# mdnunez/bayesflow_nddms

Hardware: AMD Instinct MI355X
Metric: simulated DDM trials/sec at n_trials=300 dt=0.001 (basic_ddm_dc, max_steps=4000) (higher is better)
Workload: dtype f32

## Files before the change

### bayesflow_nddms_amd/build.py

```python
import hashlib
import os
import re
import shutil
import subprocess

_HERE = os.path.dirname(os.path.abspath(__file__))
SO_PATH = os.environ.get("NDDM_HIP_LIB") or os.path.join(_HERE, "libnddm_hip.so")
SOURCES = [os.path.join(_HERE, "csrc", "nddm_kernels.hip")]
HEADERS = [os.path.join(_HERE, "csrc", "nddm_rng.h"), os.path.join(_HERE, "csrc", "nddm_sim.h"), os.path.join(_HERE, "csrc", "nddm_queue.h"),
           os.path.join(_HERE, "csrc", "nddm_prepass.h"), os.path.join(_HERE, "csrc", "nddm_ratcliff.h"),
           os.path.join(_HERE, "csrc", "nddm_wiener.h"), os.path.join(_HERE, "csrc", "nddm_wiener_cdf.h"),
           os.path.join(_HERE, "csrc", "nddm_wiener_quantile.h"), os.path.join(_HERE, "csrc", "nddm_wiener_grad.h"),
           os.path.join(_HERE, "csrc", "nddm_wiener_survival_grad.h"),
           os.path.join(_HERE, "csrc", "nddm_wiener_marginal.h"), os.path.join(_HERE, "csrc", "nddm_wiener_marginal_grad.h"),
           os.path.join(_HERE, "csrc", "nddm_wiener_hmc.h"),
           os.path.join(_HERE, "csrc", "nddm_wiener_hmc_joint.h"),
           os.path.join(os.path.dirname(_HERE), "include", "nddm.h")]
HIPCC_FLAGS = ["-O3", "-ffp-contract=off", "--offload-arch=gfx950", "-fPIC", "-shared", "-std=c++17"]


def _hipcc():
    exe = shutil.which("hipcc") or "/opt/rocm/bin/hipcc"
    if not os.path.exists(exe):
        raise RuntimeError("hipcc not found: the HIP extension cannot be built")
    return exe


def source_hash():
    h = hashlib.sha256()
    for p in SOURCES + HEADERS:
        h.update(os.path.basename(p).encode() + b"\0")
        with open(p, "rb") as f:
            h.update(f.read())
        h.update(b"\0")
    h.update(" ".join(HIPCC_FLAGS).encode())
    return h.hexdigest()


def embedded_hash(path=None):
    path = path or SO_PATH
    try:
        with open(path, "rb") as f:
            m = re.search(rb"NDDM_SRC_HASH=([0-9a-f]{64})", f.read())
    except OSError:
        return None
    return m.group(1).decode() if m else None


def is_stale():
    if os.environ.get("NDDM_HIP_LIB"):
        return False
    if not os.path.exists(SO_PATH):
        return True
    return embedded_hash() != source_hash()


def hipcc_version():
    try:
        m = re.search(r"HIP version:\s*(\S+)", subprocess.run([_hipcc(), "--version"], capture_output=True, text=True, timeout=60).stdout)
        return m.group(1) if m else "unknown"
    except Exception:
        return "unknown"


def build_hip(force=False, verbose=False):
    if not force and not is_stale():
        return SO_PATH
    import fcntl
    with open(SO_PATH + ".lock", "w") as lock:
        fcntl.flock(lock, fcntl.LOCK_EX)
        if force or is_stale():
            tmp = f"{SO_PATH}.{os.getpid()}.tmp"
            cmd = [_hipcc()] + HIPCC_FLAGS + [f'-DNDDM_SOURCE_HASH="{source_hash()}"', f'-DNDDM_HIPCC_VERSION="{hipcc_version()}"', "-o", tmp] + SOURCES
            if verbose:
                print(" ".join(cmd))
            try:
                subprocess.check_call(cmd)
                os.replace(tmp, SO_PATH)
            finally:
                if os.path.exists(tmp):
                    os.remove(tmp)
    return SO_PATH


TRAIN_SO_PATH = os.path.join(_HERE, "libnddm_train.so")
TRAIN_SOURCES = [os.path.join(_HERE, "csrc", f) for f in ("train_kernels.hip", "train_sample.hip", "train_quantile.hip", "train_deepset.hip",
                                                          "train_update.hip", "train_importance.hip", "train_wquantile.hip", "train_psis.hip")]
TRAIN_HEADERS = [os.path.join(_HERE, "csrc", f) for f in ("train_flow.h", "train_quantile.h", "train_psis.h")]
TRAIN_SOURCE = TRAIN_SOURCES[0]


def train_source_hash():
    h = hashlib.sha256()
    for path in TRAIN_SOURCES + TRAIN_HEADERS:
        with open(path, "rb") as f:
            h.update(f.read())
    return h.hexdigest()


def train_is_stale():
    stamp = TRAIN_SO_PATH + ".srchash"
    try:
        with open(stamp) as f:
            return not os.path.exists(TRAIN_SO_PATH) or f.read().strip() != train_source_hash()
    except OSError:
        return True


def build_train(force=False, verbose=False):
    if not force and not train_is_stale():
        return TRAIN_SO_PATH
    import fcntl
    with open(TRAIN_SO_PATH + ".lock", "w") as lock:
        fcntl.flock(lock, fcntl.LOCK_EX)
        if force or train_is_stale():
            tmp = f"{TRAIN_SO_PATH}.{os.getpid()}.tmp"
            cmd = [_hipcc(), "-O3", "--offload-arch=gfx950", "-std=c++17", "-fPIC", "-shared", "-o", tmp] + TRAIN_SOURCES
            if verbose:
                print(" ".join(cmd))
            try:
                subprocess.check_call(cmd)
                os.replace(tmp, TRAIN_SO_PATH)
                with open(TRAIN_SO_PATH + ".srchash", "w") as f:
                    f.write(train_source_hash())
            finally:
                if os.path.exists(tmp):
                    os.remove(tmp)
    return TRAIN_SO_PATH


if __name__ == "__main__":
    print(build_hip(force=True, verbose=True))
    print(build_train(force=True, verbose=True))
```

### bayesflow_nddms_amd/csrc/nddm_sim.h

```cpp
#pragma once
#include <hip/hip_runtime.h>
#include <math.h>
#include <stdint.h>

#include "../../include/nddm.h"
#include "nddm_queue.h"
#include "nddm_rng.h"

namespace nddm {

constexpr int WAVE = 64;
constexpr int MAX_REJECT = 64;

typedef __attribute__((address_space(3))) uint16_t lds_u16;
typedef __attribute__((address_space(3))) uint32_t lds_u32;
typedef uint32_t u32v4 __attribute__((ext_vector_type(4)));
typedef uint32_t u32v2 __attribute__((ext_vector_type(2)));
typedef __attribute__((address_space(3))) u32v4 lds_u32v4;
typedef __attribute__((address_space(3))) u32v2 lds_u32v2;

template <int MODEL> struct ModelTraits;
template <> struct ModelTraits<NDDM_BASIC_DDM_DC>      { static constexpr int P = 5; static constexpr bool HAS_Z = false; static constexpr int TAU = 3; };
template <> struct ModelTraits<NDDM_SINGLE_TRIAL>      { static constexpr int P = 8; static constexpr bool HAS_Z = true;  static constexpr int TAU = 3; };
template <> struct ModelTraits<NDDM_SINGLE_TRIAL_ALT>  { static constexpr int P = 8; static constexpr bool HAS_Z = true;  static constexpr int TAU = 3; };
template <> struct ModelTraits<NDDM_ALPHA_NOT_SCALED>  { static constexpr int P = 6; static constexpr bool HAS_Z = false; static constexpr int TAU = 3; };
template <> struct ModelTraits<NDDM_EXPLICIT_BOUNDARY> { static constexpr int P = 4; static constexpr bool HAS_Z = true;  static constexpr int TAU = 2; };

struct SimArgs {
    const float *params;
    const float *bounds;
    float *out_trials;
    float *out_summary;
    float *out_ext;
    uint16_t *out_codes;
    long long B;
    int n_trials;
    int n_total;
    int tiles_per_set;
    unsigned long long *partials;
    const uint32_t *recs;
    int max_k;
    float dt;
    float sqrt_dt;
    float tscale;
    uint32_t k0, k1;
    int sets_per_chunk;
    int n_chunks;
    unsigned int *chunk_counter;
    int ring;
    int open_ahead;
    float ext_sigma;
    int ext_mode;
    unsigned long long *dbg;
    int dbg_waves, dbg_chunks;
    int res16;
    int refill_thresh;
    uint32_t ring_magic;
    int back_from;
    double dt64, sqrt_dt64;
};

typedef const __attribute__((address_space(4))) SimArgs *ArgsPtr;
__device__ __forceinline__ ArgsPtr fresh_args(ArgsPtr p)
{
    asm volatile("" : "+s"(p));
    return p;
}

template <bool FAST>
struct AuxStream {
    uint32_t trial, set_lo, c3, blk, kbase;
    u32x4 x;
    __device__ __forceinline__ AuxStream(uint32_t kbase_, uint32_t set_lo_, uint32_t set_hi28, uint32_t trial_)
        : trial(trial_), set_lo(set_lo_), c3(set_hi28 | 0x10000000u), blk(0xffffffffu), kbase(kbase_) {}
    __device__ __forceinline__ void block(uint32_t b)
    {
        if (b != blk) { x = philox4x32_10_lds(set_lo, trial, c3, b, kbase); blk = b; }
    }
    __device__ __forceinline__ void first_pair(float &z0, float &z1)
    {
        block(0u);
        float r, cs, sn;
        polar_pair<FAST>(x.x, x.y, r, cs, sn);
        r *= noise_unit<FAST>(1.0f);
        z0 = r * cs; z1 = r * sn;
    }
    __device__ __forceinline__ float normal(uint32_t a)
    {
        block(a >> 2);
        const bool second = (a & 2u) != 0u;
        float r, cs, sn;
        polar_pair<FAST>(second ? x.z : x.x, second ? x.w : x.y, r, cs, sn);
        r *= noise_unit<FAST>(1.0f);
        return r * ((a & 1u) ? sn : cs);
    }
};

__device__ __forceinline__ unsigned long long wave_sum(unsigned long long v)
{
#pragma unroll
    for (int off = 32; off > 0; off >>= 1) v += __shfl_xor(v, off, WAVE);
    return v;
}
__device__ __forceinline__ int wave_sum(int v)
{
#pragma unroll
    for (int off = 32; off > 0; off >>= 1) v += __shfl_xor(v, off, WAVE);
    return v;
}

__device__ __forceinline__ int fresh_lane(int lane)
{
    asm volatile("" : "+v"(lane));
    return lane;
}

__device__ __forceinline__ uint32_t lane_rank(unsigned long long mask)
{
    return __builtin_amdgcn_mbcnt_hi((uint32_t)(mask >> 32), __builtin_amdgcn_mbcnt_lo((uint32_t)mask, 0u));
}

__device__ __forceinline__ void finalize_summary(float *o, int n_up, int n_lo, int n_miss, unsigned long long sk,
                                                 unsigned long long sk2, unsigned long long sk_up,
                                                 unsigned long long sk2_up, long long sz, long long szz, int n_total,
                                                 float tscale, float tau)
{
    const double dtd = (double)tscale, taud = (double)tau;
    const double n_resp = (double)(n_up + n_lo);
    o[0] = (float)n_up; o[1] = (float)n_lo; o[2] = (float)n_miss;
    if (n_resp > 0) {
        const double mk = (double)sk / n_resp;
        const double vk = (double)sk2 / n_resp - mk * mk;
        o[3] = (float)(taud + dtd * mk);
        o[4] = (float)(dtd * dtd * vk);
    } else { o[3] = __builtin_nanf(""); o[4] = __builtin_nanf(""); }
    if (n_up > 0) {
        const double nu = (double)n_up;
        const double mk = (double)sk_up / nu;
        const double vk = (double)sk2_up / nu - mk * mk;
        o[5] = (float)(taud + dtd * mk);
        o[6] = (float)(dtd * dtd * vk);
    } else { o[5] = __builtin_nanf(""); o[6] = __builtin_nanf(""); }
    const double Nd = (double)n_total;
    const double mz = ((double)sz / 4294967296.0) / Nd;
    const double vz = ((double)szz / 16777216.0) / Nd - mz * mz;
    o[7] = (float)mz;
    o[8] = (float)(vz < 0 ? 0 : vz);
    o[9] = (float)(((double)n_up + 0.5 * (double)n_miss) / Nd);
}

enum { REC = 12, R_A = 0, R_B = 4, R_SET = 8, R_TAU = 9, R_GLO = 10, R_GHI = 11 };

__device__ __forceinline__ void make_record(int model, bool fast, bool f64, const float *row, float dt, float sqrt_dt, int set,
                                            unsigned long long gset, uint32_t *r)
{
    float drift = 0.0f, a = 0.0f, beta = 0.0f, sig_c = 1.0f, tau;
    float b0 = 0.0f, b1 = 0.0f, b2 = 0.0f;
    switch (model) {
    case NDDM_BASIC_DDM_DC: drift = row[0]; a = row[1]; beta = row[2]; tau = row[3]; sig_c = row[4]; break;
    case NDDM_SINGLE_TRIAL: drift = row[0]; beta = row[2]; tau = row[3]; sig_c = row[5]; b0 = row[6]; b1 = row[7]; b2 = row[2]; break;
    case NDDM_SINGLE_TRIAL_ALT: tau = row[3]; b0 = row[5]; b1 = row[6]; b2 = row[7]; break;
    case NDDM_ALPHA_NOT_SCALED: a = row[1]; beta = row[2]; tau = row[3]; sig_c = row[5]; b0 = row[4]; break;
    default: drift = row[0]; beta = row[1]; tau = row[2]; sig_c = row[3]; break;
    }
    const float unit = sqrt_dt * sig_c;
    const float inv_s = 1.0f / (fast ? noise_unit<true>(unit) : noise_unit<false>(unit));
    const float hv = 0.5f * a;
    float a0 = (drift * dt) * inv_s, a1 = inv_s, a2 = hv * inv_s, a3 = (a * beta - hv) * inv_s;
    if (model == NDDM_SINGLE_TRIAL) { a2 = row[4]; a3 = row[1]; }
    else if (model == NDDM_SINGLE_TRIAL_ALT) { a0 = row[0]; a1 = row[1]; a2 = row[2]; a3 = row[4]; }
    else if (model == NDDM_ALPHA_NOT_SCALED) { a0 = row[0]; }
    else if (model == NDDM_EXPLICIT_BOUNDARY) { a2 = beta; a3 = 0.0f; }
    if (f64) {
        a0 = drift; a1 = sig_c;
        if (model == NDDM_BASIC_DDM_DC) { a2 = a; a3 = beta; }
    }
    r[0] = __float_as_uint(a0); r[1] = __float_as_uint(a1); r[2] = __float_as_uint(a2); r[3] = __float_as_uint(a3);
    r[4] = __float_as_uint(b0); r[5] = __float_as_uint(b1); r[6] = __float_as_uint(b2); r[7] = 0u;
    r[8] = (uint32_t)set; r[9] = __float_as_uint(tau);
    r[R_GLO] = (uint32_t)gset; r[R_GHI] = (uint32_t)(gset >> 32) & 0x0fffffffu;
}

enum { D_A = 0, D_B = 4,
       D_SIC = 8, D_TAU = 9, D_TBASE = 10, D_VSET = 11,
       D_CA = 12, D_CB = 13, D_HP1K = 14, D_X1 = 15,
       D_C3 = 16, D_SETLO = 17,
       D_ZSUM = 20,
       D_SPARE = 20 };
constexpr int DV = 24;
static_assert(D_SIC == R_SET && D_TAU == R_TAU, "the LDS record starts with the loaded record");
constexpr int LDS_HEADER_DWORDS = 32;
__host__ __device__ constexpr bool model_has_latent(int model)
{
    return model == NDDM_SINGLE_TRIAL || model == NDDM_SINGLE_TRIAL_ALT || model == NDDM_ALPHA_NOT_SCALED;
}
constexpr int LATENT_FIFO = 128;
__host__ __device__ constexpr int lds_header_bytes(int model)
{
    return LDS_HEADER_DWORDS * 4 + (model_has_latent(model) ? LATENT_FIFO * 4 : 0);
}
__host__ __device__ constexpr int slot_stride_bytes(int tile_trials, int bytes_per_result)
{
    return DV * 4 + ((tile_trials * bytes_per_result + 15) & ~15);
}

template <int MODEL, bool FAST>
__device__ __forceinline__ void trial_latent(const u32v4 dA, const u32v4 dB, uint32_t set_lo, uint32_t c3, uint32_t trial,
                                             uint32_t kbase, float &latent, float &z)
{
    static_assert(MODEL == NDDM_SINGLE_TRIAL || MODEL == NDDM_SINGLE_TRIAL_ALT, "models with a per-trial latent");
    const float sd = MODEL == NDDM_SINGLE_TRIAL ? __uint_as_float(dA.z) : __uint_as_float(dA.w);
    const float mean = MODEL == NDDM_SINGLE_TRIAL ? __uint_as_float(dA.w) : __uint_as_float(dB.x);
    const float sigma1 = MODEL == NDDM_SINGLE_TRIAL ? __uint_as_float(dB.x) : __uint_as_float(dB.y);
    const float gamma = MODEL == NDDM_SINGLE_TRIAL ? __uint_as_float(dB.y) : __uint_as_float(dB.z);
    AuxStream<FAST> aux(kbase, set_lo, c3, trial);
    float z0, z1;
    aux.first_pair(z0, z1);
    float v = __builtin_fmaf(sd, z1, mean);
    for (uint32_t ai = 2; !(v > 0.0f) && ai <= MAX_REJECT; ++ai) v = __builtin_fmaf(sd, aux.normal(ai), mean);
    if (!(v > 0.0f)) v = fabsf(v);
    latent = v;
    z = __builtin_fmaf(sigma1, z0, gamma * v);
}

template <bool FAST>
__device__ __forceinline__ float latent_normal_f64(const u32v4 dA, uint32_t set_lo, uint32_t c3, uint32_t trial, uint32_t kbase)
{
    const double sd = (double)__uint_as_float(dA.z), mean = (double)__uint_as_float(dA.w);
    AuxStream<FAST> aux(kbase, set_lo, c3, trial);
    float z0, z;
    aux.first_pair(z0, z);
    double v = mean + sd * (double)z;
    for (uint32_t ai = 2; !(v > 0.0) && ai <= MAX_REJECT; ++ai) { z = aux.normal(ai); v = mean + sd * (double)z; }
    return z;
}

__device__ __forceinline__ void z_fixed_point(float z, long long &fz, long long &fzz)
{
    z = fminf(fmaxf(z, -262144.0f), 262144.0f);
    const uint32_t b = __float_as_uint(z);
    const uint32_t e = (b >> 23) & 0xffu;
    const uint32_t m = (b & 0x007fffffu) | 0x00800000u;
    const uint32_t s1 = 147u - e, s2 = 291u - 2u * e;
    const unsigned long long mag = ((unsigned long long)m << 29) >> (s1 < 63u ? s1 : 63u);
    fz = (b >> 31) ? -(long long)mag : (long long)mag;
    fzz = (long long)((((unsigned long long)m * m) << 15) >> (s2 < 63u ? s2 : 63u));
}

template <int CTRL, int ROW_MASK>
__device__ __forceinline__ uint32_t dpp_add(uint32_t v)
{
    return v + (uint32_t)__builtin_amdgcn_update_dpp(0, (int)v, CTRL, ROW_MASK, 0xf, false);
}
__device__ __forceinline__ uint32_t wave_sum_dpp(uint32_t v)
{
    v = dpp_add<0x111, 0xf>(v);
    v = dpp_add<0x112, 0xf>(v);
    v = dpp_add<0x114, 0xf>(v);
    v = dpp_add<0x118, 0xf>(v);
    v = dpp_add<0x142, 0xa>(v);
    v = dpp_add<0x143, 0xc>(v);
    return v;
}

__host__ __device__ constexpr int partial_words(bool has_zsum) { return has_zsum ? 7 : 5; }

template <int MODEL, bool FAST, bool SMALL, bool CODES>
__device__ __forceinline__ void flush_set(ArgsPtr Ap, int lane, long long vset, uint32_t *d, const void *res, uint32_t kbase)
{
    using T = ModelTraits<MODEL>;
    constexpr bool ZSUM = MODEL == NDDM_SINGLE_TRIAL || MODEL == NDDM_SINGLE_TRIAL_ALT;
    const float tau = __uint_as_float(d[D_TAU]);
    [[maybe_unused]] u32v4 dA = {0u, 0u, 0u, 0u}, dB = {0u, 0u, 0u, 0u};
    [[maybe_unused]] uint32_t set_lo = 0u, c3 = 0u;
    [[maybe_unused]] long long acc_z = 0, acc_zz = 0;
    if constexpr (ZSUM) {
        dA = *reinterpret_cast<const u32v4 *>(d + D_A); dB = *reinterpret_cast<const u32v4 *>(d + D_B);
        c3 = d[D_C3]; set_lo = d[D_SETLO];
    }
    const int N = Ap->n_trials;
    const int TPS = Ap->tiles_per_set;
    const long long set_in_call = TPS == 1 ? vset : vset / TPS;
    const int t0 = TPS == 1 ? 0 : (int)(vset - set_in_call * TPS) * N;
    const int n_here = (Ap->n_total - t0) < N ? (Ap->n_total - t0) : N;
    uint32_t cnt2 = 0, sk32 = 0, sk2_32 = 0, sk_up32 = 0, sk2_up32 = 0;
    int n_up = 0, n_lo = 0, n_miss = 0;
    unsigned long long sk = 0, sk2 = 0, sk_up = 0, sk2_up = 0;
    float2 *out = Ap->out_trials ? reinterpret_cast<float2 *>(Ap->out_trials) + set_in_call * Ap->n_total + t0 : nullptr;
    static_assert(!CODES || (SMALL && (MODEL == NDDM_BASIC_DDM_DC || MODEL == NDDM_ALPHA_NOT_SCALED)), "wire-format kernels");
    constexpr bool HAS_CODES = CODES;
    [[maybe_unused]] uint16_t *codes = nullptr;
    if constexpr (HAS_CODES) { if (Ap->out_codes) codes = Ap->out_codes + set_in_call * Ap->n_total + t0; }
    for (uint32_t j = (uint32_t)lane; j < (uint32_t)n_here; j += WAVE) {
        uint32_t k, code;
        if (SMALL || Ap->res16) {
            const uint32_t v = static_cast<const uint16_t *>(res)[j];
            k = v & 0x3fffu; code = v >> 14;
            if constexpr (HAS_CODES) { if (codes) codes[j] = (uint16_t)v; }
        } else {
            const uint32_t v = static_cast<const uint32_t *>(res)[j];
            k = v & 0x3fffffffu; code = v >> 30;
        }
        const float ch = code == 1u ? 1.0f : (code == 2u ? -1.0f : 0.0f);
        const float rt = __builtin_fmaf((float)k, Ap->tscale, tau);
        float2 o;
        if constexpr (MODEL == NDDM_BASIC_DDM_DC) { o.x = rt; o.y = ch; }
        else if constexpr (MODEL == NDDM_ALPHA_NOT_SCALED) { o.x = ch * rt; o.y = 0.5f * (ch + 1.0f); }
        else {
            o.x = ch * rt;
            if constexpr (ZSUM) {
                float latent;
                trial_latent<MODEL, FAST>(dA, dB, set_lo, c3, (uint32_t)(t0 + j), kbase, latent, o.y);
                if (Ap->out_summary) { long long fz, fzz; z_fixed_point(o.y, fz, fzz); acc_z += fz; acc_zz += fzz; }
            } else {
                o.y = out ? Ap->bounds[set_in_call * Ap->n_total + t0 + j] : 0.0f;
            }
        }
        if constexpr (MODEL == NDDM_EXPLICIT_BOUNDARY) { if (code == 3u) o.x = __builtin_nanf(""); }
        if (out) out[j] = o;
        if (Ap->out_summary) {
            if constexpr (SMALL) {
                const uint32_t up01 = __builtin_amdgcn_ubfe(0x2u, code, 1u), resp01 = __builtin_amdgcn_ubfe(0x6u, code, 1u);
                const uint32_t kr = __umul24(k, resp01), ku = __umul24(k, up01);
                cnt2 += up01 | (resp01 << 10);
                sk32 += kr; sk_up32 += ku;
                sk2_32 = __umul24(kr, k) + sk2_32; sk2_up32 = __umul24(ku, k) + sk2_up32;
            } else {
                const unsigned long long kk = (unsigned long long)k * k;
                if (code == 1u) { n_up++; sk += k; sk2 += kk; sk_up += k; sk2_up += kk; }
                else if (code == 2u) { n_lo++; sk += k; sk2 += kk; }
                else n_miss++;
            }
        }
    }
    if (Ap->out_summary) {
        unsigned long long *q = reinterpret_cast<unsigned long long *>(Ap->partials) + vset * partial_words(ZSUM);
        [[maybe_unused]] unsigned long long *zsum = reinterpret_cast<unsigned long long *>(d + D_ZSUM);
        if constexpr (ZSUM) {
            atomicAdd(zsum, (unsigned long long)acc_z);
            atomicAdd(zsum + 1, (unsigned long long)acc_zz);
        }
        if constexpr (SMALL) {
            cnt2 = wave_sum_dpp(cnt2);
            sk32 = wave_sum_dpp(sk32); sk_up32 = wave_sum_dpp(sk_up32);
            const uint32_t a_hi = wave_sum_dpp(sk2_32 >> 16), a_lo = wave_sum_dpp(sk2_32 & 0xffffu);
            const uint32_t u_hi = wave_sum_dpp(sk2_up32 >> 16), u_lo = wave_sum_dpp(sk2_up32 & 0xffffu);
            if (fresh_lane(lane) == WAVE - 1) {
                const uint32_t n_up = cnt2 & 1023u, n_resp = cnt2 >> 10;
                q[0] = (unsigned long long)n_up | ((unsigned long long)(n_resp - n_up) << 21) |
                       ((unsigned long long)((uint32_t)n_here - n_resp) << 42);
                q[1] = sk32; q[2] = ((unsigned long long)a_hi << 16) + a_lo;
                q[3] = sk_up32; q[4] = ((unsigned long long)u_hi << 16) + u_lo;
                if constexpr (ZSUM) { q[5] = zsum[0]; q[6] = zsum[1]; }
            }
        } else {
            n_up = wave_sum(n_up); n_lo = wave_sum(n_lo); n_miss = wave_sum(n_miss);
            sk = wave_sum(sk); sk2 = wave_sum(sk2); sk_up = wave_sum(sk_up); sk2_up = wave_sum(sk2_up);
            if (fresh_lane(lane) == 0) {
                q[0] = (unsigned long long)n_up | ((unsigned long long)n_lo << 21) | ((unsigned long long)n_miss << 42);
                q[1] = sk; q[2] = sk2; q[3] = sk_up; q[4] = sk2_up;
                if constexpr (ZSUM) { q[5] = zsum[0]; q[6] = zsum[1]; }
            }
        }
    }
    if constexpr (MODEL == NDDM_ALPHA_NOT_SCALED) {
        if (Ap->out_ext && fresh_lane(lane) == 0 && t0 == 0) {
            AuxStream<FAST> aux(kbase, d[D_SETLO], d[D_C3], 0xffffffffu);
            const float loc = (Ap->ext_mode == 0) ? Ap->params[set_in_call * T::P + 1] : 1.0f;
            Ap->out_ext[set_in_call] = __builtin_fmaf(Ap->ext_sigma, aux.normal(0), loc);
        }
    }
}

__device__ __forceinline__ int ring_slot(int t, int ring, uint32_t magic)
{
    const uint32_t q = (uint32_t)(((unsigned long long)(uint32_t)t * magic) >> 32);
    int r = t - (int)(q * (uint32_t)ring);
    return r >= ring ? r - ring : r;
}

__device__ __forceinline__ bool in_range(float w, float h)
{
    return __builtin_fabsf(w) < h;
}


template <int MODEL, bool FAST, bool CAP4, bool BRIDGE, bool SMALL, bool PACKED, bool VKEYS, bool CODES = false, bool F64 = false>
__global__ __launch_bounds__(WAVE) void sim_kernel(const SimArgs A)
{
    static_assert(!F64 || ((MODEL == NDDM_BASIC_DDM_DC || MODEL == NDDM_SINGLE_TRIAL) && !BRIDGE && !PACKED && !VKEYS && !CODES),
                  "NDDM_STATE_F64 kernels");
    using T = ModelTraits<MODEL>;
    constexpr int P = T::P;
    extern __shared__ uint32_t lds_raw[];

    const ArgsPtr Ak = (ArgsPtr)__builtin_amdgcn_kernarg_segment_ptr();
    const int lane = threadIdx.x;
    const int N = A.n_trials;

    if (lane < 10) { lds_raw[2 * lane] = A.k0 + (uint32_t)lane * 0x9E3779B9u; lds_raw[2 * lane + 1] = A.k1 + (uint32_t)lane * 0xBB67AE85u; }
    if (lane == 0) { lds_raw[28] = A.k0 + 2u * PHILOX_W0; lds_raw[29] = A.k1 + 2u * PHILOX_W1; lds_raw[30] = A.k0 + 3u * PHILOX_W0; }
    uint32_t kbase;
    {
        const uint32_t off = (uint32_t)(size_t)lds_raw;
        asm volatile("v_mov_b32 %0, %1" : "=v"(kbase) : "s"(off));
    }
    const int rshift = SMALL ? 1 : (BRIDGE ? 2 : (A.res16 ? 1 : 2));
    constexpr bool LATENT = model_has_latent(MODEL);
    const int stride = DV * 4 + (((N << rshift) + 15) & ~15);
    char *const slots = reinterpret_cast<char *>(lds_raw) + lds_header_bytes(MODEL);
    auto slot_rec = [&](int slot) { return reinterpret_cast<uint32_t *>(slots + slot * stride); };
    auto pack_slots = [&](int t) {
        const ArgsPtr R = fresh_args(Ak);
        const int s0 = ring_slot(t, R->ring, R->ring_magic);
        const int o0 = s0 * stride, o01 = (s0 + 1 == R->ring ? 0 : s0 + 1) * stride - o0;
        return (o0 & 0xffff) | (o01 << 16);
    };
    constexpr uint32_t SLOTS_OFF = lds_header_bytes(MODEL);
    constexpr uint32_t FIFO_OFF = LDS_HEADER_DWORDS * 4;
    [[maybe_unused]] int fifo_pos = 0, fifo_avail = 0;

    float w = 0.0f, h = 0.0f, mu_dt = 0.0f;
    [[maybe_unused]] double xe = 0.0, ab = 0.0, cdt = 0.0, sdc = 0.0;
    int k = 0;
    [[maybe_unused]] float ta = 0.0f, tb = 0.0f;
    [[maybe_unused]] uint32_t jraw = 0;
    uint32_t res_addr = 0;
    [[maybe_unused]] int tile = 0;
    bool invalid = false;
    unsigned long long has_m = 0ull, act_m = 0ull;
    constexpr int MAX_BLOCKS = 16;
    [[maybe_unused]] int cap_k = -1;
    PathCtr pc = {0u, 0u, 0u, 0u, 0u};
    [[maybe_unused]] PathKeys pkeys;
    if constexpr (VKEYS) pkeys.init(A.k0, A.k1);

    int tile_open = 0;
    int flushed = 0;
    int next_tile = 0, next_trial = 0;
    int to_retire = N;
    int chunk_set = 0, chunk_left = 0;
    int slot_pack = pack_slots(0);
    int dirty = 1;
    unsigned long long dbg_cnt = 0;
    unsigned long long *dbg_stamp = reinterpret_cast<unsigned long long *>(lds_raw + 20);
    if (lane == 0) {
        dbg_stamp[3] = 0;
        lds_raw[31] = blockIdx.x;
        if (Ak->dbg) { dbg_stamp[0] = __builtin_amdgcn_s_memtime(); dbg_stamp[1] = __builtin_amdgcn_s_memrealtime(); }
    }

    uint32_t pre = 0u;

    auto open_tiles = [&]() {
        const ArgsPtr R = fresh_args(Ak);
        while (tile_open < flushed + R->ring && tile_open <= next_tile + R->open_ahead) {
            const bool have_pre = chunk_left > 0;
            if (chunk_left <= 0) {
                if (chunk_left < 0) break;
                const bool from_back = __builtin_amdgcn_readfirstlane((int)lds_raw[31]) >= R->back_from;
                unsigned long long old = 0ull;
                if (fresh_lane(lane) == 0)
                    old = atomicAdd(reinterpret_cast<unsigned long long *>(R->chunk_counter), from_back ? QUEUE_BACK : QUEUE_FRONT);
                old = ((unsigned long long)(uint32_t)__builtin_amdgcn_readfirstlane((int)(old >> 32)) << 32) |
                      (uint32_t)__builtin_amdgcn_readfirstlane((int)(uint32_t)old);
                const long long pulled = queue_pull(old, R->n_chunks, from_back);
                const unsigned int c = (unsigned int)pulled;
                if (pulled < 0) {
                    chunk_left = -1;
                    if (fresh_lane(lane) == 0 && R->dbg) dbg_stamp[3] = __builtin_amdgcn_s_memrealtime();
                    break;
                }
                if (fresh_lane(lane) == 0 && R->dbg && c < (unsigned int)R->dbg_chunks)
                    R->dbg[8ll * R->dbg_waves + c] = __builtin_amdgcn_s_memrealtime();
                chunk_set = (int)c * R->sets_per_chunk;
                const long long left = R->B - (long long)chunk_set;
                chunk_left = (int)(left < R->sets_per_chunk ? left : R->sets_per_chunk);
            }
            const int slot = ring_slot(tile_open, R->ring, R->ring_magic);
            const int TPS = R->tiles_per_set;
            const int prow = TPS == 1 ? chunk_set : chunk_set / TPS;
            const int qt = chunk_set - prow * TPS;
            uint32_t rec = pre;
            if (!have_pre) rec = fresh_lane(lane) < REC ? R->recs[(long long)prow * REC + lane] : 0u;
            if (chunk_left > 1) {
                const int nrow = TPS == 1 ? chunk_set + 1 : (chunk_set + 1) / TPS;
                if (nrow != prow) pre = fresh_lane(lane) < REC ? R->recs[(long long)nrow * REC + lane] : 0u;
                else pre = rec;
            }
            const int sic = __builtin_amdgcn_readlane((int)rec, R_SET);
            const int vset = sic * TPS + qt;
            uint32_t *d = slot_rec(slot);
            if (lane < REC) d[lane] = rec;
            const uint32_t s_lo = (uint32_t)__builtin_amdgcn_readlane((int)rec, R_GLO);
            const uint32_t s_hi = (uint32_t)__builtin_amdgcn_readlane((int)rec, R_GHI);
            if (lane == 0) {
                d[D_VSET] = (uint32_t)vset;
                if constexpr (MODEL == NDDM_SINGLE_TRIAL || MODEL == NDDM_SINGLE_TRIAL_ALT) { d[D_ZSUM] = 0u; d[D_ZSUM + 1] = 0u; d[D_ZSUM + 2] = 0u; d[D_ZSUM + 3] = 0u; }
                PathSet ps;
                ps.init(s_lo, s_hi, R->k0, R->k1);
                d[D_CA] = ps.cA; d[D_CB] = ps.cB; d[D_HP1K] = ps.hP1k; d[D_X1] = ps.X1;
                d[D_SETLO] = s_lo;
                d[D_C3] = s_hi;
                d[D_TBASE] = (uint32_t)(qt * N);
            }
            chunk_set++; chunk_left--; tile_open++;
        }
    };

    while (true) {
        const unsigned long long fin_mask0 = has_m & ~act_m;
        if (__builtin_amdgcn_inverse_ballot_w64(fin_mask0)) {
            uint32_t code = invalid ? 3u : (w >= h ? 1u : (w <= -h ? 2u : 0u));
            if constexpr (F64) code = xe >= ab ? 1u : (xe <= 0.0 ? 2u : 0u);
            uint32_t tfix = (uint32_t)k;
            if constexpr (BRIDGE) {
                const bool started = fmaxf(ta, tb) > 0.0f;
                const bool stepped = started && k < A.max_k;
                code = (stepped || !started) ? (w >= 0.0f ? 1u : 2u) : 0u;
                const uint32_t jit = (k & 1) ? ((jraw >> 16) & 0xffu) : (jraw & 0xffu);
                tfix = (((uint32_t)k + (stepped ? 1u : 0u)) << 8) - (stepped ? jit : 0u);
            }
            if (SMALL || rshift == 1) *reinterpret_cast<lds_u16 *>(res_addr + (SLOTS_OFF + DV * 4)) = (uint16_t)(tfix | (code << 14));
            else *reinterpret_cast<lds_u32 *>(res_addr + (SLOTS_OFF + DV * 4)) = tfix | (code << 30);
        }
        has_m &= ~fin_mask0;
        to_retire -= (int)__popcll(fin_mask0);
        if (to_retire <= 0) {
            __syncthreads();
            while (flushed < tile_open) {
                if (next_tile <= flushed) break;
                const int fslot = ring_slot(flushed, fresh_args(Ak)->ring, fresh_args(Ak)->ring_magic);
                if constexpr (SMALL) {
                    const uint32_t fsb = (uint32_t)(fslot * stride) + kbase;
                    if (__builtin_amdgcn_ballot_w64(res_addr - fsb < (uint32_t)stride) & has_m) break;
                } else {
                    if (__builtin_amdgcn_ballot_w64(tile == flushed) & has_m) break;
                }
                uint32_t *const d = slot_rec(fslot);
                const int set_in_call = __builtin_amdgcn_readfirstlane((int)d[D_VSET]);
                flush_set<MODEL, FAST, SMALL, CODES>(fresh_args(Ak), lane, (long long)set_in_call, d, d + DV, kbase);
                flushed++;
                to_retire += N;
                dirty = 1;
            }
            __syncthreads();
        }
        if (dirty) {
            dirty = 0;
            if (tile_open <= next_tile + fresh_args(Ak)->open_ahead && tile_open < flushed + fresh_args(Ak)->ring && chunk_left >= 0) {
                open_tiles();
                __syncthreads();
            }
            if (flushed == tile_open && chunk_left < 0) break;
        }
        {
            const unsigned long long want_mask = ~has_m;
            int tr = next_trial + (int)lane_rank(want_mask);
            int tl = next_tile;
            while (tr >= N) { tr -= N; tl++; }
            const unsigned long long ok_mask = want_mask & __builtin_amdgcn_ballot_w64(tl < tile_open);
            const int off0 = slot_pack & 0xffff, off01 = slot_pack >> 16;
            const int tile0 = next_tile;
            if constexpr (LATENT) {
                const int n_ok = (int)__popcll(ok_mask);
                if (n_ok > fifo_avail) {
                    int btr = next_trial + fifo_avail + lane, btl = next_tile;
                    while (btr >= N) { btr -= N; btl++; }
                    const unsigned long long bmask = __builtin_amdgcn_ballot_w64(btl < tile_open);
                    if (__builtin_amdgcn_inverse_ballot_w64(bmask)) {
                        const uint32_t bsb = (uint32_t)(__mul24(btl - tile0, off01) + off0) + kbase;
                        const lds_u32v4 *const bq = reinterpret_cast<const lds_u32v4 *>(bsb + SLOTS_OFF);
                        const u32v4 dA = bq[D_A / 4];
                        [[maybe_unused]] const u32v4 dB = bq[D_B / 4];
                        const u32v4 dS = bq[D_SIC / 4];
                        const u32v2 sw = *reinterpret_cast<const lds_u32v2 *>(bsb + SLOTS_OFF + D_C3 * 4);
                        const uint32_t btrial = (uint32_t)btr + dS.z;
                        float v;
                        if constexpr (MODEL == NDDM_ALPHA_NOT_SCALED) {
                            AuxStream<FAST> aux(kbase, sw.y, sw.x, btrial);
                            v = (__builtin_fmaf(__uint_as_float(dB.x), aux.normal(0), __uint_as_float(dA.x)) * fresh_args(Ak)->dt) * __uint_as_float(dA.y);
                        } else if constexpr (F64) {
                            v = latent_normal_f64<FAST>(dA, sw.y, sw.x, btrial, kbase);
                        } else {
                            float z_unused;
                            trial_latent<MODEL, FAST>(dA, dB, sw.y, sw.x, btrial, kbase, v, z_unused);
                        }
                        *reinterpret_cast<__attribute__((address_space(3))) float *>(
                            kbase + FIFO_OFF + (((uint32_t)(fifo_pos + fifo_avail + lane) & (LATENT_FIFO - 1)) << 2)) = v;
                    }
                    fifo_avail += (int)__popcll(bmask);
                }
            }
            next_trial += (int)__popcll(ok_mask);
            if (next_trial >= N) {
                const int ring_bytes = fresh_args(Ak)->ring * stride;
                int o0 = slot_pack & 0xffff, o01 = slot_pack >> 16;
                while (next_trial >= N) {
                    next_trial -= N; next_tile++;
                    o0 += o01;
                    o01 = o0 + stride == ring_bytes ? -o0 : stride;
                }
                slot_pack = (o0 & 0xffff) | (o01 << 16);
                dirty = 1;
            }
            has_m |= ok_mask;
            if (__builtin_amdgcn_inverse_ballot_w64(ok_mask)) {
#ifdef NDDM_EXTRA_REFILL_VALU
                { uint32_t dummy = (uint32_t)lane;
#pragma unroll
                  for (int e = 0; e < NDDM_EXTRA_REFILL_VALU; ++e) asm volatile("v_xor_b32 %0, 0x55, %0" : "+v"(dummy)); }
#endif
                const ArgsPtr H = fresh_args(Ak);
                if constexpr (!SMALL) tile = tl;
                const uint32_t sb = (uint32_t)(__mul24(tl - tile0, off01) + off0) + kbase;
                res_addr = sb + ((uint32_t)tr << rshift);
                const lds_u32v4 *const rq = reinterpret_cast<const lds_u32v4 *>(sb + SLOTS_OFF);
                const lds_u32 *const rw = reinterpret_cast<const lds_u32 *>(sb + SLOTS_OFF);
                const u32v4 d0 = rq[D_A / 4];
                const u32v4 d1 = rq[D_CA / 4];
                const u32v4 d2 = rq[D_SIC / 4];
                const float a0 = __uint_as_float(d0.x), a1 = __uint_as_float(d0.y), a2 = __uint_as_float(d0.z),
                            a3 = __uint_as_float(d0.w);
                const uint32_t trial = (uint32_t)tr + d2.z;
                [[maybe_unused]] float latent = 0.0f;
                if constexpr (LATENT)
                    latent = *reinterpret_cast<const __attribute__((address_space(3))) float *>(
                        kbase + FIFO_OFF + (((uint32_t)fifo_pos + lane_rank(want_mask)) & (LATENT_FIFO - 1)) * 4u);
                invalid = false;
                if constexpr (F64) {
                    double beta64;
                    if constexpr (MODEL == NDDM_BASIC_DDM_DC) { ab = (double)a2; beta64 = (double)a3; }
                    else {
                        ab = (double)a3 + (double)a2 * (double)latent;
                        if (!(ab > 0.0)) ab = __builtin_fabs(ab);
                        beta64 = (double)__uint_as_float(rw[D_B + 2]);
                    }
                    xe = ab * beta64;
                    cdt = (double)a0 * H->dt64;
                    sdc = H->sqrt_dt64 * (double)a1;
                    if constexpr (FAST) sdc *= 1.1774100225154747;
                } else if constexpr (MODEL == NDDM_BASIC_DDM_DC) {
                    mu_dt = a0; h = a2; w = a3;
                } else if constexpr (MODEL == NDDM_SINGLE_TRIAL) {
                    const float a = latent;
                    const float hv = 0.5f * a;
                    mu_dt = a0;
                    h = hv * a1;
                    w = (a * __uint_as_float(rw[D_B + 2]) - hv) * a1;
                } else if constexpr (MODEL == NDDM_SINGLE_TRIAL_ALT) {
                    const float sig_c = latent;
                    const float inv_t = 1.0f / noise_unit<FAST>(H->sqrt_dt * sig_c);
                    const float hv = 0.5f * a1;
                    mu_dt = (a0 * H->dt) * inv_t;
                    h = hv * inv_t;
                    w = (a1 * a2 - hv) * inv_t;
                } else if constexpr (MODEL == NDDM_ALPHA_NOT_SCALED) {
                    mu_dt = latent;
                    h = a2; w = a3;
                } else if constexpr (MODEL == NDDM_EXPLICIT_BOUNDARY) {
                    const float a = trial < (uint32_t)H->n_total ? H->bounds[(long long)d2.x * H->n_total + trial] : 1.0f;
                    invalid = !(a >= 0.0f);
                    const float hv = 0.5f * a;
                    mu_dt = a0;
                    h = invalid ? 0.0f : hv * a1;
                    w = (a * a2 - hv) * a1;
                }
                const uint4 kq = *reinterpret_cast<const uint4 *>(lds_raw + 28);
                pc.init(d1.x, d1.y, d1.z, d1.w, trial, kq.x, kq.y, kq.z);
                k = 0;
                if constexpr (BRIDGE) { ta = h - __builtin_fabsf(w); tb = ta; jraw = 0u; }
            }
            if constexpr (LATENT) { const int n_ok = (int)__popcll(ok_mask); fifo_pos += n_ok; fifo_avail -= n_ok; }
            if constexpr (BRIDGE) act_m = __builtin_amdgcn_ballot_w64(ta > 0.0f) & __builtin_amdgcn_ballot_w64(k < A.max_k) & has_m;
            else if constexpr (F64) act_m = __builtin_amdgcn_ballot_w64(xe > 0.0) & __builtin_amdgcn_ballot_w64(xe < ab) & __builtin_amdgcn_ballot_w64(k < A.max_k) & has_m;
            else if constexpr (CAP4 && !PACKED) {
                const int max_k = fresh_args(Ak)->max_k;
                act_m = max_k > 0 ? __builtin_amdgcn_ballot_w64(in_range(w, h)) & has_m : 0ull;
                const int near_from = A.refill_thresh < WAVE ? max_k - 4 * MAX_BLOCKS : (int)0x80000000;
                cap_k = (__builtin_amdgcn_ballot_w64(k >= near_from) & has_m) ? max_k : -1;
            }
            else act_m = __builtin_amdgcn_ballot_w64(in_range(w, h)) & __builtin_amdgcn_ballot_w64(k < A.max_k) & has_m;
        }
        const int it_limit = A.refill_thresh < WAVE ? MAX_BLOCKS - 1 : 0x7fffffff;
        const int occupied = (int)__popcll(has_m);
        const int leave_at = occupied < A.refill_thresh ? occupied : A.refill_thresh;
        int it = 0;
        for (;; ++it) {
            if constexpr (BRIDGE) {
                const uint32_t blk = (uint32_t)k;
                const u32x4 u4 = philox4x32_10_path(blk | 0x80000000u, pc, kbase);
                unsigned long long &live = act_m;
#pragma unroll
                for (int half = 0; half < 2; ++half) {
                    const u32x4 rb = philox4x32_10_path(blk + 4u * (uint32_t)half, pc, kbase);
                    float r0, r1, c0, c1, c2, c3;
                    polar_pair<FAST, true>(rb.x, rb.y, r0, c0, c1);
                    polar_pair<FAST, true>(rb.z, rb.w, r1, c2, c3);
                    const uint32_t ua = half ? u4.z : u4.x, ub = half ? u4.w : u4.y;
                    if constexpr (FAST && CAP4) {
                        float m, uf;
#define NDDM_BSTEP(R, T, D0, D1, CVT, KLIT) "v_fmac_f32 %[w], %[" R "], %[" T "]\n\tv_add_f32 %[w], %[mu], %[w]\n\tv_sub_f32 %[" D1 "], %[h], |%[w]|\n\t" \
    "v_mul_f32 %[m], %[" D0 "], %[" D1 "]\n\tv_fmaak_f32 %[m], -4.0, %[m], " KLIT "\n\tv_exp_f32 %[m], %[m]\n\t" CVT                        \
    "v_cmpx_ge_f32_e64 vcc, %[uf], %[m]\n\tv_add_u32 %[k], 1, %[k]\n\t"
#define NDDM_U32(W) "v_cvt_f32_u32 %[uf], %[" W "]\n\t"
#define NDDM_U16(W) "v_and_b32 %[uf], 0xffff, %[" W "]\n\tv_cvt_f32_u32 %[uf], %[uf]\n\t"
                        asm volatile("s_mov_b64 exec, %[lm]\n\t"
                                     "v_mov_b32 %[jr], %[ua]\n\t"
                                     NDDM_BSTEP("r0", "c0", "ta", "tb", NDDM_U32("ua"), "0x42000001")
                                     NDDM_BSTEP("r0", "c1", "tb", "ta", NDDM_U16("ua"), "0x41800000")
                                     "v_mov_b32 %[jr], %[ub]\n\t"
                                     NDDM_BSTEP("r1", "c2", "ta", "tb", NDDM_U32("ub"), "0x42000001")
                                     NDDM_BSTEP("r1", "c3", "tb", "ta", NDDM_U16("ub"), "0x41800000")
                                     "s_nop 1\n\ts_mov_b64 %[lm], exec\n\ts_mov_b64 exec, -1"
                                     : [w] "+v"(w), [k] "+v"(k), [ta] "+v"(ta), [tb] "+v"(tb), [jr] "+v"(jraw), [lm] "+s"(live), [m] "=&v"(m),
                                       [uf] "=&v"(uf)
                                     : [mu] "v"(mu_dt), [h] "v"(h), [r0] "v"(r0), [r1] "v"(r1), [c0] "v"(c0), [c1] "v"(c1),
                                       [c2] "v"(c2), [c3] "v"(c3), [ua] "v"(ua), [ub] "v"(ub)
                                     : "vcc");
#undef NDDM_BSTEP
#undef NDDM_U32
#undef NDDM_U16
                    } else {
                        bool active = __builtin_amdgcn_inverse_ballot_w64(live);
                        const float rr4[4] = {r0, r0, r1, r1}, tt4[4] = {c0, c1, c2, c3};
#pragma unroll
                        for (int j = 0; j < 4; ++j) {
                            if (active) {
                                asm volatile("" ::: "memory");
                                const uint32_t word = j < 2 ? ua : ub;
                                const float w1 = __builtin_fmaf(rr4[j], tt4[j], w) + mu_dt;
                                const float t1 = h - __builtin_fabsf(w1);
                                const float m = ((j & 1) ? tb : ta) * t1;
                                if (j & 1) ta = t1; else tb = t1;
                                if ((j & 1) == 0) jraw = word;
                                const float uf = (j & 1) ? (float)(word & 0xffffu) : (float)word;
                                bool cross;
                                if constexpr (FAST) {
                                    const float kk = (j & 1) ? 16.0f : __uint_as_float(0x42000001u);
                                    cross = !(uf >= __builtin_amdgcn_exp2f(__builtin_fmaf(-4.0f, m, kk)));
                                } else {
                                    const float u = uf * ((j & 1) ? 1.52587890625e-05f : 2.3283064365386963e-10f);
                                    cross = !(t1 > 0.0f) || u < exact_expf_neg(-2.0f * m);
                                }
                                w = w1;
                                if (cross) active = false;
                                else {
                                    k++;
                                    if constexpr (!CAP4) active = k < A.max_k;
                                }
                            }
                        }
                        live = __builtin_amdgcn_ballot_w64(active);
                    }
                }
                act_m &= __builtin_amdgcn_ballot_w64(k < A.max_k);
                if ((int)__popcll(has_m & ~act_m) >= leave_at) break;
                if (it >= it_limit) break;
                continue;
            }
            [[maybe_unused]] bool active = (CAP4 && !PACKED && !F64) ? false : __builtin_amdgcn_inverse_ballot_w64(act_m);
            constexpr int NS = PACKED ? 8 : 4;
            const uint32_t blk = (uint32_t)k;
            u32x4 rb;
            if constexpr (VKEYS) rb = philox4x32_10_path(blk, pc, pkeys);
            else rb = philox4x32_10_path(blk, pc, kbase);
            float rr[NS], tt[NS];
            if constexpr (PACKED) {
                polar_pair_packed<FAST>(rb.x, rr[0], tt[0], tt[1]);
                polar_pair_packed<FAST>(rb.y, rr[2], tt[2], tt[3]);
                polar_pair_packed<FAST>(rb.z, rr[4], tt[4], tt[5]);
                polar_pair_packed<FAST>(rb.w, rr[6], tt[6], tt[7]);
                rr[1] = rr[0]; rr[3] = rr[2]; rr[5] = rr[4]; rr[7] = rr[6];
            } else {
                polar_pair<FAST, true>(rb.x, rb.y, rr[0], tt[0], tt[1]);
                polar_pair<FAST, true>(rb.z, rb.w, rr[2], tt[2], tt[3]);
                rr[1] = rr[0]; rr[3] = rr[2];
            }
            if constexpr (F64) {
#pragma unroll
                for (int j = 0; j < NS; ++j) {
                    if (active) {
                        asm volatile("" ::: "memory");
                        const double zn = (double)rr[j] * (double)tt[j];
                        xe = xe + (cdt + sdc * zn);
                        k++;
                        if (j < NS - 1) {
                            if constexpr (CAP4) active = (xe > 0.0) && (xe < ab);
                            else active = (xe > 0.0) && (xe < ab) && (k < A.max_k);
                        }
                    }
                }
                act_m = __builtin_amdgcn_ballot_w64(xe > 0.0) & __builtin_amdgcn_ballot_w64(xe < ab) & __builtin_amdgcn_ballot_w64(k < A.max_k) & has_m;
                if ((int)__popcll(has_m & ~act_m) >= leave_at) break;
                if (it >= it_limit) break;
                continue;
            }
            if constexpr (CAP4 && !PACKED) {
#define NDDM_STEP(R, T, K2) "v_fmac_f32 %[w], %[" R "], %[" T "]\n\tv_add_f32 %[w], %[mu], %[w]\n\t" K2 "v_cmpx_lt_f32_e64 vcc, |%[w]|, %[h]\n\t"
#define NDDM_K2 "v_add_u32 %[k], 2, %[k]\n\t"
                asm volatile("s_mov_b64 exec, %[am]\n\t"
                             NDDM_STEP("r0", "t0", NDDM_K2) "s_xor_b64 %[am], %[am], vcc\n\t"
                             NDDM_STEP("r0", "t1", "")      "s_xor_b64 %[am], %[am], vcc\n\t"
                             NDDM_STEP("r1", "t2", NDDM_K2) "s_xor_b64 %[am], %[am], vcc\n\t"
                             NDDM_STEP("r1", "t3", "")      "s_andn2_b64 %[am], %[am], vcc\n\t"
                             "s_cbranch_scc0 1f\n\t"
                             "s_mov_b64 exec, %[am]\n\t"
                             "v_subrev_u32 %[k], 1, %[k]\n"
                             "1:\n\t"
                             "s_mov_b64 %[am], vcc\n\t"
                             "s_mov_b64 exec, -1\n\t"
                             "s_cmp_lt_i32 %[ck], 0\n\t"
                             "s_cbranch_scc1 2f\n\t"
                             "v_cmp_gt_i32 vcc, %[ck], %[k]\n\t"
                             "s_and_b64 %[am], %[am], vcc\n"
                             "2:"
                             : [w] "+v"(w), [k] "+v"(k), [am] "+s"(act_m)
                             : [ck] "s"(cap_k), [mu] "v"(mu_dt), [h] "v"(h), [r0] "v"(rr[0]), [r1] "v"(rr[2]),
                               [t0] "v"(tt[0]), [t1] "v"(tt[1]), [t2] "v"(tt[2]), [t3] "v"(tt[3])
                             : "vcc", "scc");
#undef NDDM_STEP
#undef NDDM_K2
                if ((int)__popcll(has_m & ~act_m) >= leave_at) break;
                if (it >= it_limit) break;
                continue;
            }
#pragma unroll
            for (int j = 0; j < NS; ++j) {
                if (active) {
                    asm volatile("" ::: "memory");
                    w = __builtin_fmaf(rr[j], tt[j], w) + mu_dt;
                    k++;
                    if (j < NS - 1) {
                        if constexpr (CAP4) active = in_range(w, h);
                        else active = in_range(w, h) && (k < A.max_k);
                    }
                }
            }
            act_m = __builtin_amdgcn_ballot_w64(in_range(w, h)) & __builtin_amdgcn_ballot_w64(k < A.max_k) & has_m;
            if ((int)__popcll(has_m & ~act_m) >= leave_at) break;
            if (it >= it_limit) break;
        }
        dbg_cnt += (1ull << 32) | (unsigned long long)(uint32_t)(it + 1);
    }
    if (lane == 0) {
        unsigned int *const q = fresh_args(Ak)->chunk_counter;
        const unsigned int left = atomicAdd(q + 2, 1u);
        if (left == gridDim.x - 1u) { atomicExch(reinterpret_cast<unsigned long long *>(q), 0ull); atomicExch(q + 2, 0u); }
    }
    unsigned long long *const dbg = fresh_args(Ak)->dbg;
    if (dbg && lane == 0) {
        const unsigned long long t_end = __builtin_amdgcn_s_memrealtime(), c_end = __builtin_amdgcn_s_memtime();
        const uint32_t wg = lds_raw[31];
        if (wg < (uint32_t)fresh_args(Ak)->dbg_waves) {
            unsigned long long *const r = dbg + 8ull * wg;
            r[0] = dbg_cnt & 0xffffffffull; r[1] = dbg_cnt >> 32;
            r[2] = c_end - dbg_stamp[0]; r[3] = t_end - dbg_stamp[1];
            r[4] = dbg_stamp[1]; r[5] = dbg_stamp[3]; r[6] = t_end; r[7] = 1ull;
        }
    }
}

}
```

Measured before the change: 9.688 billion.

## Latch exit-step parity bits to drop per-block exit fixup branch in CAP4 stepping

Adds an exit latch for CAP4 small kernels. The inner 4-step asm block accumulates a parity mask (lat_b0) in place of the old andn2/conditional-branch k fixup. The finish path then writes the 16-bit result code and step count with a single masked ds_write computed in asm. A rare-case scalar path corrects lanes that left through the cap or NaN conditions. This removes a scalar branch and exec juggling from the hot stepping loop, in exchange for more complex finish logic and the risk of wrong step counts in edge cases.

```diff
diff --git a/bayesflow_nddms_amd/build.py b/bayesflow_nddms_amd/build.py
--- a/bayesflow_nddms_amd/build.py
+++ b/bayesflow_nddms_amd/build.py
@@ -8,6 +8,7 @@
 SO_PATH = os.environ.get("NDDM_HIP_LIB") or os.path.join(_HERE, "libnddm_hip.so")
 SOURCES = [os.path.join(_HERE, "csrc", "nddm_kernels.hip")]
 HEADERS = [os.path.join(_HERE, "csrc", "nddm_rng.h"), os.path.join(_HERE, "csrc", "nddm_sim.h"), os.path.join(_HERE, "csrc", "nddm_queue.h"),
+           os.path.join(_HERE, "csrc", "nddm_exit_latch.h"),
            os.path.join(_HERE, "csrc", "nddm_prepass.h"), os.path.join(_HERE, "csrc", "nddm_ratcliff.h"),
            os.path.join(_HERE, "csrc", "nddm_wiener.h"), os.path.join(_HERE, "csrc", "nddm_wiener_cdf.h"),
            os.path.join(_HERE, "csrc", "nddm_wiener_quantile.h"), os.path.join(_HERE, "csrc", "nddm_wiener_grad.h"),
diff --git a/bayesflow_nddms_amd/csrc/nddm_exit_latch.h b/bayesflow_nddms_amd/csrc/nddm_exit_latch.h
--- /dev/null
+++ b/bayesflow_nddms_amd/csrc/nddm_exit_latch.h
@@ -0,0 +1,54 @@
+#pragma once
+
+namespace nddm {
+
+#if defined(__HIPCC__)
+#define NDDM_LATCH_FN __host__ __device__ __forceinline__
+#else
+#define NDDM_LATCH_FN inline
+#endif
+
+typedef unsigned long long latch_mask;
+
+struct ExitLatch {
+    latch_mask b0, b1, left;
+};
+
+NDDM_LATCH_FN latch_mask latch_b0(latch_mask b0, latch_mask m1, latch_mask m2, latch_mask m3, latch_mask m4)
+{
+    return b0 ^ m1 ^ m2 ^ m3 ^ m4;
+}
+
+NDDM_LATCH_FN latch_mask latch_b1(latch_mask b1, latch_mask m2, latch_mask m4)
+{
+    return b1 ^ m2 ^ m4;
+}
+
+NDDM_LATCH_FN latch_mask latch_l(latch_mask left, latch_mask am, latch_mask m4)
+{
+    return left | (am & ~m4);
+}
+
+NDDM_LATCH_FN void latch_block(ExitLatch &s, latch_mask am, latch_mask m1, latch_mask m2, latch_mask m3, latch_mask m4)
+{
+    s.b0 = latch_b0(s.b0, m1, m2, m3, m4);
+    s.b1 = latch_b1(s.b1, m2, m4);
+    s.left = latch_l(s.left, am, m4);
+}
+
+NDDM_LATCH_FN latch_mask latch_left(latch_mask am_first, latch_mask m4_last, latch_mask capped)
+{
+    return am_first & ~m4_last & ~capped;
+}
+
+NDDM_LATCH_FN int latch_exit_step(bool b0, bool b1)
+{
+    return 1 + (b0 ? 1 : 0) + (b1 ? 2 : 0);
+}
+
+NDDM_LATCH_FN int latch_step_of_pair(int k_pair, bool b0)
+{
+    return k_pair - 1 + (b0 ? 1 : 0);
+}
+
+}
diff --git a/bayesflow_nddms_amd/csrc/nddm_sim.h b/bayesflow_nddms_amd/csrc/nddm_sim.h
--- a/bayesflow_nddms_amd/csrc/nddm_sim.h
+++ b/bayesflow_nddms_amd/csrc/nddm_sim.h
@@ -4,6 +4,7 @@
 #include <stdint.h>
 
 #include "../../include/nddm.h"
+#include "nddm_exit_latch.h"
 #include "nddm_queue.h"
 #include "nddm_rng.h"
 
@@ -385,6 +386,14 @@
 }
 
 
+
+__host__ __device__ constexpr bool exit_latch_kernel(int model, bool fast, bool cap4, bool bridge, bool small, bool packed, bool codes, bool f64)
+{
+    if (!cap4 || bridge || packed || f64 || !small) return false;
+    if (model == NDDM_ALPHA_NOT_SCALED && codes && !fast) return false;
+    return model != NDDM_SINGLE_TRIAL && model != NDDM_SINGLE_TRIAL_ALT;
+}
+
 template <int MODEL, bool FAST, bool CAP4, bool BRIDGE, bool SMALL, bool PACKED, bool VKEYS, bool CODES = false, bool F64 = false>
 __global__ __launch_bounds__(WAVE) void sim_kernel(const SimArgs A)
 {
@@ -392,6 +401,7 @@
                   "NDDM_STATE_F64 kernels");
     using T = ModelTraits<MODEL>;
     constexpr int P = T::P;
+    constexpr bool LATCH = exit_latch_kernel(MODEL, FAST, CAP4, BRIDGE, SMALL, PACKED, CODES, F64);
     extern __shared__ uint32_t lds_raw[];
 
     const ArgsPtr Ak = (ArgsPtr)__builtin_amdgcn_kernarg_segment_ptr();
@@ -431,6 +441,7 @@
     unsigned long long has_m = 0ull, act_m = 0ull;
     constexpr int MAX_BLOCKS = 16;
     [[maybe_unused]] int cap_k = -1;
+    [[maybe_unused]] unsigned long long lat_b0 = 0ull, act_first = 0ull;
     PathCtr pc = {0u, 0u, 0u, 0u, 0u};
     [[maybe_unused]] PathKeys pkeys;
     if constexpr (VKEYS) pkeys.init(A.k0, A.k1);
@@ -510,7 +521,38 @@
 
     while (true) {
         const unsigned long long fin_mask0 = has_m & ~act_m;
-        if (__builtin_amdgcn_inverse_ballot_w64(fin_mask0)) {
+        if constexpr (LATCH) {
+            unsigned long long rare;
+            {
+                uint32_t word;
+                asm volatile("v_cmp_o_f32 vcc, %[w], %[w]\n\t"
+                             "s_cmp_lt_i32 %[ck], 0\n\t"
+                             "s_cselect_b64 %[rare], %[af], 0\n\t"
+                             "s_andn2_b64 %[rare], %[rare], %[am]\n\t"
+                             "s_and_b64 %[rare], %[rare], vcc\n\t"
+                             "s_andn2_b64 %[rare], %[fin], %[rare]\n\t"
+                             "v_lshrrev_b32 %[t], 31, %[w]\n\t"
+                             "v_lshl_add_u32 %[t], %[t], 14, %[k]\n\t"
+                             "s_mov_b64 vcc, %[b0]\n\t"
+                             "v_addc_co_u32 %[t], vcc, %[c], %[t], vcc\n\t"
+                             "s_xor_b64 exec, %[fin], %[rare]\n\t"
+                             "ds_write_b16 %[ra], %[t] offset:%[off]\n\t"
+                             "s_mov_b64 exec, -1"
+                             : [t] "=&v"(word), [rare] "=&s"(rare)
+                             : [w] "v"(w), [k] "v"(k), [c] "v"(0x3fffu), [b0] "s"(lat_b0), [fin] "s"(fin_mask0),
+                               [af] "s"(act_first), [am] "s"(act_m), [ck] "s"(cap_k), [ra] "v"(res_addr), [off] "n"(SLOTS_OFF + DV * 4)
+                             : "vcc", "scc", "memory");
+            }
+            if (rare) {
+                const unsigned long long left = latch_left(act_first, act_m, __builtin_amdgcn_ballot_w64(in_range(w, h)));
+                if (__builtin_amdgcn_inverse_ballot_w64(rare)) {
+                    const uint32_t code = invalid ? 3u : (w >= h ? 1u : (w <= -h ? 2u : 0u));
+                    uint32_t tfix = (uint32_t)k;
+                    if (__builtin_amdgcn_inverse_ballot_w64(left)) tfix = (uint32_t)latch_step_of_pair(k, __builtin_amdgcn_inverse_ballot_w64(lat_b0));
+                    *reinterpret_cast<lds_u16 *>(res_addr + (SLOTS_OFF + DV * 4)) = (uint16_t)(tfix | (code << 14));
+                }
+            }
+        } else if (__builtin_amdgcn_inverse_ballot_w64(fin_mask0)) {
             uint32_t code = invalid ? 3u : (w >= h ? 1u : (w <= -h ? 2u : 0u));
             if constexpr (F64) code = xe >= ab ? 1u : (xe <= 0.0 ? 2u : 0u);
             uint32_t tfix = (uint32_t)k;
@@ -679,6 +721,7 @@
                 act_m = max_k > 0 ? __builtin_amdgcn_ballot_w64(in_range(w, h)) & has_m : 0ull;
                 const int near_from = A.refill_thresh < WAVE ? max_k - 4 * MAX_BLOCKS : (int)0x80000000;
                 cap_k = (__builtin_amdgcn_ballot_w64(k >= near_from) & has_m) ? max_k : -1;
+                if constexpr (LATCH) { lat_b0 = 0ull; act_first = act_m; }
             }
             else act_m = __builtin_amdgcn_ballot_w64(in_range(w, h)) & __builtin_amdgcn_ballot_w64(k < A.max_k) & has_m;
         }
@@ -799,6 +842,24 @@
             if constexpr (CAP4 && !PACKED) {
 #define NDDM_STEP(R, T, K2) "v_fmac_f32 %[w], %[" R "], %[" T "]\n\tv_add_f32 %[w], %[mu], %[w]\n\t" K2 "v_cmpx_lt_f32_e64 vcc, |%[w]|, %[h]\n\t"
 #define NDDM_K2 "v_add_u32 %[k], 2, %[k]\n\t"
+                if constexpr (LATCH)
+                    asm volatile("s_mov_b64 exec, %[am]\n\t"
+                                 NDDM_STEP("r0", "t0", NDDM_K2) "s_xor_b64 %[b0], %[b0], vcc\n\t"
+                                 NDDM_STEP("r0", "t1", "")      "s_xor_b64 %[b0], %[b0], vcc\n\t"
+                                 NDDM_STEP("r1", "t2", NDDM_K2) "s_xor_b64 %[b0], %[b0], vcc\n\t"
+                                 NDDM_STEP("r1", "t3", "")      "s_xor_b64 %[b0], %[b0], vcc\n\t"
+                                 "s_mov_b64 %[am], vcc\n\t"
+                                 "s_mov_b64 exec, -1\n\t"
+                                 "s_cmp_lt_i32 %[ck], 0\n\t"
+                                 "s_cbranch_scc1 2f\n\t"
+                                 "v_cmp_gt_i32 vcc, %[ck], %[k]\n\t"
+                                 "s_and_b64 %[am], %[am], vcc\n"
+                                 "2:"
+                                 : [w] "+v"(w), [k] "+v"(k), [am] "+s"(act_m), [b0] "+s"(lat_b0)
+                                 : [ck] "s"(cap_k), [mu] "v"(mu_dt), [h] "v"(h), [r0] "v"(rr[0]), [r1] "v"(rr[2]),
+                                   [t0] "v"(tt[0]), [t1] "v"(tt[1]), [t2] "v"(tt[2]), [t3] "v"(tt[3])
+                                 : "vcc", "scc");
+                else
                 asm volatile("s_mov_b64 exec, %[am]\n\t"
                              NDDM_STEP("r0", "t0", NDDM_K2) "s_xor_b64 %[am], %[am], vcc\n\t"
                              NDDM_STEP("r0", "t1", "")      "s_xor_b64 %[am], %[am], vcc\n\t"
```

New measurement: 9.709 billion, median of 6. Within noise of the previous version (+0.2%).
